# iwbn/flow-supervisor

Hardware: AMD Instinct MI355X
Metric: image-pairs/s fwd+bwd, 12 GRU iters, 436x1024 (higher is better)
Workload: dtype f32 (bf16x3 products); 1 GPU; RAFT full, 440x1024 (Sintel 436x1024 padded), 12 GRU iters, 4 pairs/GPU, train step = fwd + sequence loss + bwd + RCCL all-reduce + clip + AdamW; global_batch=4, parallelism=dp1, launch=hipGraph replay of the whole step

## Files before the change

flow_supervisor_amd/csrc/conv_pack.hip:

```cpp
#include "conv_common.hpp"

namespace {

struct PackArgs {
  float* w;
  float* wpk;
  int Cout, Cin, taps;
  int C[3]; int nsrc;
  int Ktot, rows;
  int mode, accumulate;
  int split;
};

__device__ __forceinline__ void store_packed(const PackArgs& a, int64_t e, float v) {
  if (!a.split) { a.wpk[e] = v; return; }
  const __bf16 h = (__bf16)v;
  const __bf16 l = (__bf16)(v - (float)h);
  __bf16* rec = reinterpret_cast<__bf16*>(a.wpk) + (e >> 5) * 64;
  rec[e & 31] = h;
  rec[32 + (e & 31)] = l;
}

__global__ __launch_bounds__(256) void pack_weight_kernel(PackArgs a) {
  const int64_t total = (int64_t)a.rows * a.Ktot;
  for (int64_t e = (int64_t)blockIdx.x * 256 + threadIdx.x; e < total; e += (int64_t)gridDim.x * 256) {
    const int n = (int)(e / a.Ktot);
    int k = (int)(e % a.Ktot);
    if (a.mode == 1) {
      const int cpad = ((a.Cout + 31) / 32) * 32;
      const int tp = k / cpad, c = k % cpad;
      float v = 0.f;
      if (c < a.Cout && n < a.Cin) v = a.w[((int64_t)c * a.Cin + n) * a.taps + (a.taps - 1 - tp)];
      store_packed(a, e, v);
    } else {
      int s = 0, coff = 0;
      for (; s < a.nsrc; ++s) {
        const int span = a.taps * (((a.C[s] + 31) / 32) * 32);
        if (k < span) break;
        k -= span; coff += a.C[s];
      }
      const int cpad = ((a.C[s] + 31) / 32) * 32;
      const int t = k / cpad, c = k % cpad;
      const bool ok = c < a.C[s] && n < a.Cout;
      if (a.mode == 0) {
        store_packed(a, e, ok ? a.w[((int64_t)n * a.Cin + coff + c) * a.taps + t] : 0.f);
      } else if (ok) {
        float* d = a.w + ((int64_t)n * a.Cin + coff + c) * a.taps + t;
        *d = a.accumulate ? *d + a.wpk[e] : a.wpk[e];
      }
    }
  }
}

using PackJob = fsraft_pack_job;
constexpr int PACK_JOBS = 16;
struct PackJobs { fsraft_pack_job j[PACK_JOBS]; };

__device__ __forceinline__ float* pack_elem(const PackJob& j, int n, int s, int c, int t) {
  int p = 0;
  while (p + 1 < j.npiece && n >= j.rows[p]) { n -= j.rows[p]; ++p; }
  float* w = j.w[p];
  if (j.flags & 2) {
    const int C = j.cin_full;
    const int sp = c / C, c0 = c % C;
    const int ky = 2 * (t >> 1) + (sp >> 1) - 1, kx = 2 * (t & 1) + (sp & 1) - 1;
    if (ky < 0 || kx < 0) return nullptr;
    return w + ((int64_t)n * C + c0) * 9 + ky * 3 + kx;
  }
  return w + ((int64_t)n * j.cin_full + j.srcOff[s] + c) * (j.kh * j.kw) + t;
}

__device__ __forceinline__ void pack_store(const PackJob& j, int Ktot, int rows, int n, int k, float v) {
  const int64_t e = (int64_t)n * Ktot + k;
  if (j.mode < 10) { j.wpk[e] = v; return; }
  const __bf16 h = (__bf16)v;
  const __bf16 l = (__bf16)(v - (float)h);
  __bf16* out = reinterpret_cast<__bf16*>(j.wpk);
  if (!(j.flags & 1)) {
    __bf16* rec = out + (e >> 5) * 64;
    rec[e & 31] = h;
    rec[32 + (e & 31)] = l;
    return;
  }
  const int nb = (rows + 31) / 32, kt = k >> 5, q = k & 31;
  const int64_t base = (((int64_t)kt * nb + (n >> 5)) * 2) ;
  const int sidx = (q >> 4) & 1, kh2 = (q >> 3) & 1, dw = (q >> 1) & 3, half = q & 1;
  const int64_t dh = ((((base + 0) * 2 + sidx) * 2 + kh2) * 32 + (n & 31)) * 4 + dw;
  const int64_t dl = ((((base + 1) * 2 + sidx) * 2 + kh2) * 32 + (n & 31)) * 4 + dw;
  out[dh * 2 + half] = h;
  out[dl * 2 + half] = l;
}

__global__ __launch_bounds__(256) void pack_jobs_kernel(PackJobs tab) {
  const PackJob& j = tab.j[blockIdx.y];
  const int taps = j.kh * j.kw;
  int cout = 0;
  for (int p = 0; p < j.npiece; ++p) cout += j.rows[p];
  if (j.mode == 3) {
    for (int e = blockIdx.x * 256 + threadIdx.x; e < cout; e += gridDim.x * 256) {
      int n = e, p = 0;
      while (p + 1 < j.npiece && n >= j.rows[p]) { n -= j.rows[p]; ++p; }
      j.wpk[e] = j.w[p][n];
    }
    return;
  }
  int cin = 0;
  for (int s = 0; s < j.nsrc; ++s) cin += j.srcC[s];
  const int m = j.mode % 10;
  int Ktot, rows;
  if (m == 1) { Ktot = taps * ((cout + 31) / 32 * 32); rows = cin; }
  else { Ktot = 0; for (int s = 0; s < j.nsrc; ++s) Ktot += taps * ((j.srcC[s] + 31) / 32 * 32); rows = cout; }
  const int rows_out = (j.flags & 1) ? (rows + 31) / 32 * 32 : rows;
  const int64_t total = (int64_t)rows_out * Ktot;
  for (int64_t e = (int64_t)blockIdx.x * 256 + threadIdx.x; e < total; e += (int64_t)gridDim.x * 256) {
    const int n = (int)(e / Ktot);
    int k = (int)(e % Ktot);
    if (m == 1) {
      const int cpad = (cout + 31) / 32 * 32;
      const int tp = k / cpad, c = k % cpad;
      float v = 0.f;
      if (c < cout && n < rows) {
        int s = 0, cs = n;
        while (s + 1 < j.nsrc && cs >= j.srcC[s]) { cs -= j.srcC[s]; ++s; }
        const float* q = pack_elem(j, c, s, cs, taps - 1 - tp);
        if (q) v = *q;
      }
      pack_store(j, Ktot, rows, n, k, v);
    } else {
      const int k0 = k;
      int s = 0;
      for (; s < j.nsrc; ++s) {
        const int span = taps * ((j.srcC[s] + 31) / 32 * 32);
        if (k < span) break;
        k -= span;
      }
      const int cpad = (j.srcC[s] + 31) / 32 * 32;
      const int t = k / cpad, c = k % cpad;
      const bool ok = c < j.srcC[s] && n < rows;
      float* q = ok ? pack_elem(j, n, s, c, t) : nullptr;
      if (m == 0) pack_store(j, Ktot, rows, n, k0, q ? *q : 0.f);
      else if (q) *q = j.accumulate ? *q + j.scale * j.wpk[e] : j.scale * j.wpk[e];
    }
  }
}

}

extern "C" int fsraft_pack_conv_weights(const fsraft_pack_job* jobs, int njobs, hipStream_t stream) {
  if (njobs < 0 || (njobs && !jobs)) return FS_ERR_ARG;
  for (int i = 0; i < njobs; ++i) {
    const fsraft_pack_job& j = jobs[i];
    const int m = j.mode;
    if (!(m == 0 || m == 1 || m == 2 || m == 3 || m == 10 || m == 11) || !j.wpk || j.npiece < 1 || j.npiece > 3) return FS_ERR_ARG;
    for (int p = 0; p < j.npiece; ++p) if (!j.w[p] || j.rows[p] < 1) return FS_ERR_ARG;
    if (m == 3) continue;
    if (j.nsrc < 1 || j.nsrc > 3 || j.kh < 1 || j.kw < 1 || j.cin_full < 1) return FS_ERR_ARG;
    if ((j.flags & 1) && m < 10) return FS_ERR_ARG;
    if ((j.flags & 2) && (j.kh != 2 || j.kw != 2 || j.nsrc != 1 || j.srcC[0] != 4 * j.cin_full || j.srcOff[0] != 0)) return FS_ERR_ARG;
    if (!(j.flags & 2)) for (int s = 0; s < j.nsrc; ++s) if (j.srcC[s] < 1 || j.srcOff[s] < 0 || j.srcOff[s] + j.srcC[s] > j.cin_full) return FS_ERR_ARG;
  }
  for (int i0 = 0; i0 < njobs; i0 += PACK_JOBS) {
    PackJobs tab{};
    const int n = njobs - i0 < PACK_JOBS ? njobs - i0 : PACK_JOBS;
    int64_t most = 0;
    for (int i = 0; i < n; ++i) {
      tab.j[i] = jobs[i0 + i];
      const fsraft_pack_job& j = tab.j[i];
      int64_t cout = 0, cin = 0;
      for (int p = 0; p < j.npiece; ++p) cout += j.rows[p];
      for (int s = 0; s < j.nsrc; ++s) cin += (j.srcC[s] + 31) / 32 * 32;
      const int64_t tot = j.mode == 3 ? cout : ((cout + 31) / 32 * 32) * ((cin + 31) / 32 * 32) * j.kh * j.kw;
      most = tot > most ? tot : most;
    }
    int blocks = (int)((most + 1023) / 1024);
    blocks = blocks < 1 ? 1 : (blocks > 512 ? 512 : blocks);
    hipLaunchKernelGGL(pack_jobs_kernel, dim3(blocks, n), dim3(256), 0, stream, tab);
  }
  return fs_launch_status();
}

extern "C" int fsraft_pack_conv_weight(float* w_oihw, float* wpk, int Cout, int Cin, int KH, int KW, const int* srcC,
                                       int nsrc, int mode, int accumulate, hipStream_t stream) {
  if (!w_oihw || !wpk || mode < 0 || (mode > 2 && mode != 10 && mode != 11)) return FS_ERR_ARG;
  PackArgs a{};
  a.split = mode >= 10;
  if (mode >= 10) mode -= 10;
  if (a.split && mode > 1) return FS_ERR_ARG;
  a.w = w_oihw; a.wpk = wpk; a.Cout = Cout; a.Cin = Cin; a.taps = KH * KW; a.mode = mode; a.accumulate = accumulate;
  if (mode == 1) {
    a.nsrc = 1; a.C[0] = Cout; a.C[1] = a.C[2] = 0;
    a.Ktot = a.taps * (((Cout + 31) / 32) * 32);
    a.rows = Cin;
  } else {
    if (!srcC || nsrc < 1 || nsrc > 3) return FS_ERR_ARG;
    int tot = 0;
    for (int s = 0; s < 3; ++s) { a.C[s] = s < nsrc ? srcC[s] : 0; tot += a.C[s]; }
    if (tot != Cin) return FS_ERR_ARG;
    a.nsrc = nsrc;
    a.Ktot = conv_ktot(srcC, nsrc, a.taps);
    a.rows = Cout;
  }
  const int64_t total = (int64_t)a.rows * a.Ktot;
  int blocks = (int)((total + 255) / 256 < 4096 ? (total + 255) / 256 : 4096);
  hipLaunchKernelGGL(pack_weight_kernel, dim3(blocks), dim3(256), 0, stream, a);
  return fs_launch_status();
}
```

Before: 111.1 image-pairs/s.

## Pack conv weights per 32-element record with vectorized stores and flat job grid

```diff
diff --git a/flow_supervisor_amd/csrc/conv_pack.hip b/flow_supervisor_amd/csrc/conv_pack.hip
--- a/flow_supervisor_amd/csrc/conv_pack.hip
+++ b/flow_supervisor_amd/csrc/conv_pack.hip
@@ -1,4 +1,5 @@
 #include "conv_common.hpp"
+#include <climits>
 
 namespace {
 
@@ -52,96 +53,149 @@
   }
 }
 
-using PackJob = fsraft_pack_job;
-constexpr int PACK_JOBS = 16;
-struct PackJobs { fsraft_pack_job j[PACK_JOBS]; };
-
-__device__ __forceinline__ float* pack_elem(const PackJob& j, int n, int s, int c, int t) {
-  int p = 0;
-  while (p + 1 < j.npiece && n >= j.rows[p]) { n -= j.rows[p]; ++p; }
-  float* w = j.w[p];
-  if (j.flags & 2) {
+constexpr int PACK_JOBS = 40;
+constexpr int PACK_RECS = 64;
+
+struct PackRec {
+  float* w[3];
+  float* wpk;
+  int rowEnd[3];
+  int cin_full, taps;
+  int srcC[3], srcOff[3];
+  int bits;
+  float scale;
+};
+struct PackTab {
+  PackRec j[PACK_JOBS];
+  int first[PACK_JOBS];
+  int njobs;
+};
+static_assert(sizeof(PackTab) <= 3840, "the job table has to fit the kernel argument segment");
+
+__device__ __forceinline__ int pick3(const int* a, int i) { return i == 0 ? a[0] : (i == 1 ? a[1] : a[2]); }
+__device__ __forceinline__ int ceil32(int v) { return (v + 31) / 32 * 32; }
+
+__device__ __forceinline__ float* pack_elem(const PackRec& j, int n, int s, int c, int t) {
+  const int p = (n >= j.rowEnd[0]) + (n >= j.rowEnd[1]);
+  float* w = p == 0 ? j.w[0] : (p == 1 ? j.w[1] : j.w[2]);
+  n -= p == 0 ? 0 : (p == 1 ? j.rowEnd[0] : j.rowEnd[1]);
+  if (j.bits & (2 << 7)) {
     const int C = j.cin_full;
     const int sp = c / C, c0 = c % C;
     const int ky = 2 * (t >> 1) + (sp >> 1) - 1, kx = 2 * (t & 1) + (sp & 1) - 1;
     if (ky < 0 || kx < 0) return nullptr;
     return w + ((int64_t)n * C + c0) * 9 + ky * 3 + kx;
   }
-  return w + ((int64_t)n * j.cin_full + j.srcOff[s] + c) * (j.kh * j.kw) + t;
-}
-
-__device__ __forceinline__ void pack_store(const PackJob& j, int Ktot, int rows, int n, int k, float v) {
-  const int64_t e = (int64_t)n * Ktot + k;
-  if (j.mode < 10) { j.wpk[e] = v; return; }
-  const __bf16 h = (__bf16)v;
-  const __bf16 l = (__bf16)(v - (float)h);
-  __bf16* out = reinterpret_cast<__bf16*>(j.wpk);
-  if (!(j.flags & 1)) {
-    __bf16* rec = out + (e >> 5) * 64;
-    rec[e & 31] = h;
-    rec[32 + (e & 31)] = l;
+  return w + ((int64_t)n * j.cin_full + pick3(j.srcOff, s) + c) * j.taps + t;
+}
+
+__device__ __forceinline__ uint32_t bf16_pair(__bf16 a, __bf16 b) {
+  return (uint32_t)__builtin_bit_cast(unsigned short, a) | ((uint32_t)__builtin_bit_cast(unsigned short, b) << 16);
+}
+
+__global__ __launch_bounds__(256) void pack_records_kernel(PackTab tab) {
+  const int blk = blockIdx.x;
+  int ji = 0, hi = tab.njobs - 1;
+  while (ji < hi) {
+    const int mid = (ji + hi + 1) >> 1;
+    if (tab.first[mid] <= blk) ji = mid; else hi = mid - 1;
+  }
+  const PackRec& j = tab.j[ji];
+  const int64_t r = (int64_t)(blk - tab.first[ji]) * PACK_RECS + (threadIdx.x >> 2);
+  const int l = threadIdx.x & 3;
+  const int nsrc = j.bits & 3, m = (j.bits >> 4) & 3, taps = j.taps, cout = j.rowEnd[2];
+  const bool split = j.bits & (1 << 6), frag = j.bits & (1 << 7), acc = j.bits & (1 << 9);
+  if (m == 3) {
+    for (int i = 0; i < 8; ++i) {
+      const int64_t e = r * 32 + l * 8 + i;
+      if (e >= cout) break;
+      const int n = (int)e, p = (n >= j.rowEnd[0]) + (n >= j.rowEnd[1]);
+      const float* w = p == 0 ? j.w[0] : (p == 1 ? j.w[1] : j.w[2]);
+      j.wpk[e] = w[n - (p == 0 ? 0 : (p == 1 ? j.rowEnd[0] : j.rowEnd[1]))];
+    }
     return;
   }
-  const int nb = (rows + 31) / 32, kt = k >> 5, q = k & 31;
-  const int64_t base = (((int64_t)kt * nb + (n >> 5)) * 2) ;
-  const int sidx = (q >> 4) & 1, kh2 = (q >> 3) & 1, dw = (q >> 1) & 3, half = q & 1;
-  const int64_t dh = ((((base + 0) * 2 + sidx) * 2 + kh2) * 32 + (n & 31)) * 4 + dw;
-  const int64_t dl = ((((base + 1) * 2 + sidx) * 2 + kh2) * 32 + (n & 31)) * 4 + dw;
-  out[dh * 2 + half] = h;
-  out[dl * 2 + half] = l;
-}
-
-__global__ __launch_bounds__(256) void pack_jobs_kernel(PackJobs tab) {
-  const PackJob& j = tab.j[blockIdx.y];
-  const int taps = j.kh * j.kw;
-  int cout = 0;
+  int cin = 0, kfwd = 0;
+  for (int s = 0; s < nsrc; ++s) { cin += pick3(j.srcC, s); kfwd += taps * ceil32(pick3(j.srcC, s)); }
+  const int cpo = ceil32(cout);
+  const int Ktot = m == 1 ? taps * cpo : kfwd, rows = m == 1 ? cin : cout;
+  const int rows_out = frag ? ceil32(rows) : rows;
+  const int KT = Ktot >> 5;
+  if (r >= (int64_t)rows_out * KT) return;
+  float* q[8];
+  int n, kt;
+  if (m == 1) {
+    const int per = rows_out * taps, ct = (int)(r / per), rem = (int)(r % per);
+    n = rem / taps;
+    const int tp = rem % taps;
+    kt = tp * (cpo >> 5) + ct;
+    int s = 0, cs = n;
+    while (s + 1 < nsrc && cs >= pick3(j.srcC, s)) { cs -= pick3(j.srcC, s); ++s; }
+    for (int i = 0; i < 8; ++i) {
+      const int c = ct * 32 + l * 8 + i;
+      q[i] = (c < cout && n < rows) ? pack_elem(j, c, s, cs, taps - 1 - tp) : nullptr;
+    }
+  } else {
+    n = (int)(r / KT);
+    kt = (int)(r % KT);
+    int k = kt * 32 + l * 8, s = 0;
+    for (; s + 1 < nsrc; ++s) {
+      const int span = taps * ceil32(pick3(j.srcC, s));
+      if (k < span) break;
+      k -= span;
+    }
+    const int cs = pick3(j.srcC, s), cpad = ceil32(cs);
+    const int t = k / cpad, c0 = k % cpad;
+    for (int i = 0; i < 8; ++i) q[i] = (c0 + i < cs && n < rows) ? pack_elem(j, n, s, c0 + i, t) : nullptr;
+  }
+  const int64_t e = (int64_t)n * Ktot + kt * 32 + l * 8;
+  if (m == 2) {
+    const float4 a = *reinterpret_cast<const float4*>(j.wpk + e), b = *reinterpret_cast<const float4*>(j.wpk + e + 4);
+    const float x[8] = {a.x, a.y, a.z, a.w, b.x, b.y, b.z, b.w};
+    for (int i = 0; i < 8; ++i)
+      if (q[i]) *q[i] = acc ? *q[i] + j.scale * x[i] : j.scale * x[i];
+    return;
+  }
+  float v[8];
+  for (int i = 0; i < 8; ++i) v[i] = q[i] ? *q[i] : 0.f;
+  if (!split) {
+    *reinterpret_cast<float4*>(j.wpk + e) = make_float4(v[0], v[1], v[2], v[3]);
+    *reinterpret_cast<float4*>(j.wpk + e + 4) = make_float4(v[4], v[5], v[6], v[7]);
+    return;
+  }
+  uint32_t h[4], lo[4];
+  for (int i = 0; i < 4; ++i) {
+    const __bf16 h0 = (__bf16)v[2 * i], h1 = (__bf16)v[2 * i + 1];
+    const __bf16 l0 = (__bf16)(v[2 * i] - (float)h0), l1 = (__bf16)(v[2 * i + 1] - (float)h1);
+    h[i] = bf16_pair(h0, h1);
+    lo[i] = bf16_pair(l0, l1);
+  }
+  uint32_t* out = reinterpret_cast<uint32_t*>(j.wpk);
+  int64_t dh, dl;
+  if (!frag) {
+    dh = (e >> 5) * 32 + l * 4;
+    dl = dh + 16;
+  } else {
+    const int nb = (rows + 31) / 32;
+    const int64_t base = ((int64_t)kt * nb + (n >> 5)) * 2;
+    dh = (((base + 0) * 4 + l) * 32 + (n & 31)) * 4;
+    dl = (((base + 1) * 4 + l) * 32 + (n & 31)) * 4;
+  }
+  *reinterpret_cast<uint4*>(out + dh) = make_uint4(h[0], h[1], h[2], h[3]);
+  *reinterpret_cast<uint4*>(out + dl) = make_uint4(lo[0], lo[1], lo[2], lo[3]);
+}
+
+int64_t pack_job_blocks(const fsraft_pack_job& j) {
+  int64_t cout = 0, cin = 0, kfwd = 0;
   for (int p = 0; p < j.npiece; ++p) cout += j.rows[p];
-  if (j.mode == 3) {
-    for (int e = blockIdx.x * 256 + threadIdx.x; e < cout; e += gridDim.x * 256) {
-      int n = e, p = 0;
-      while (p + 1 < j.npiece && n >= j.rows[p]) { n -= j.rows[p]; ++p; }
-      j.wpk[e] = j.w[p][n];
-    }
-    return;
-  }
-  int cin = 0;
-  for (int s = 0; s < j.nsrc; ++s) cin += j.srcC[s];
-  const int m = j.mode % 10;
-  int Ktot, rows;
-  if (m == 1) { Ktot = taps * ((cout + 31) / 32 * 32); rows = cin; }
-  else { Ktot = 0; for (int s = 0; s < j.nsrc; ++s) Ktot += taps * ((j.srcC[s] + 31) / 32 * 32); rows = cout; }
-  const int rows_out = (j.flags & 1) ? (rows + 31) / 32 * 32 : rows;
-  const int64_t total = (int64_t)rows_out * Ktot;
-  for (int64_t e = (int64_t)blockIdx.x * 256 + threadIdx.x; e < total; e += (int64_t)gridDim.x * 256) {
-    const int n = (int)(e / Ktot);
-    int k = (int)(e % Ktot);
-    if (m == 1) {
-      const int cpad = (cout + 31) / 32 * 32;
-      const int tp = k / cpad, c = k % cpad;
-      float v = 0.f;
-      if (c < cout && n < rows) {
-        int s = 0, cs = n;
-        while (s + 1 < j.nsrc && cs >= j.srcC[s]) { cs -= j.srcC[s]; ++s; }
-        const float* q = pack_elem(j, c, s, cs, taps - 1 - tp);
-        if (q) v = *q;
-      }
-      pack_store(j, Ktot, rows, n, k, v);
-    } else {
-      const int k0 = k;
-      int s = 0;
-      for (; s < j.nsrc; ++s) {
-        const int span = taps * ((j.srcC[s] + 31) / 32 * 32);
-        if (k < span) break;
-        k -= span;
-      }
-      const int cpad = (j.srcC[s] + 31) / 32 * 32;
-      const int t = k / cpad, c = k % cpad;
-      const bool ok = c < j.srcC[s] && n < rows;
-      float* q = ok ? pack_elem(j, n, s, c, t) : nullptr;
-      if (m == 0) pack_store(j, Ktot, rows, n, k0, q ? *q : 0.f);
-      else if (q) *q = j.accumulate ? *q + j.scale * j.wpk[e] : j.scale * j.wpk[e];
-    }
-  }
+  if (j.mode == 3) return ((cout + 31) / 32 + PACK_RECS - 1) / PACK_RECS;
+  const int64_t taps = (int64_t)j.kh * j.kw;
+  for (int s = 0; s < j.nsrc; ++s) { cin += j.srcC[s]; kfwd += taps * ((j.srcC[s] + 31) / 32); }
+  const bool dgrad = j.mode % 10 == 1;
+  int64_t rows = dgrad ? cin : cout;
+  if (j.flags & 1) rows = (rows + 31) / 32 * 32;
+  const int64_t recs = rows * (dgrad ? taps * ((cout + 31) / 32) : kfwd);
+  return (recs + PACK_RECS - 1) / PACK_RECS;
 }
 
 }
@@ -158,23 +212,32 @@
     if ((j.flags & 1) && m < 10) return FS_ERR_ARG;
     if ((j.flags & 2) && (j.kh != 2 || j.kw != 2 || j.nsrc != 1 || j.srcC[0] != 4 * j.cin_full || j.srcOff[0] != 0)) return FS_ERR_ARG;
     if (!(j.flags & 2)) for (int s = 0; s < j.nsrc; ++s) if (j.srcC[s] < 1 || j.srcOff[s] < 0 || j.srcOff[s] + j.srcC[s] > j.cin_full) return FS_ERR_ARG;
+    if ((reinterpret_cast<uintptr_t>(j.wpk) & 15) || (int64_t)j.kh * j.kw > (1 << 20) || pack_job_blocks(j) > INT_MAX / 2) return FS_ERR_ARG;
   }
   for (int i0 = 0; i0 < njobs; i0 += PACK_JOBS) {
-    PackJobs tab{};
-    const int n = njobs - i0 < PACK_JOBS ? njobs - i0 : PACK_JOBS;
-    int64_t most = 0;
-    for (int i = 0; i < n; ++i) {
-      tab.j[i] = jobs[i0 + i];
-      const fsraft_pack_job& j = tab.j[i];
-      int64_t cout = 0, cin = 0;
-      for (int p = 0; p < j.npiece; ++p) cout += j.rows[p];
-      for (int s = 0; s < j.nsrc; ++s) cin += (j.srcC[s] + 31) / 32 * 32;
-      const int64_t tot = j.mode == 3 ? cout : ((cout + 31) / 32 * 32) * ((cin + 31) / 32 * 32) * j.kh * j.kw;
-      most = tot > most ? tot : most;
-    }
-    int blocks = (int)((most + 1023) / 1024);
-    blocks = blocks < 1 ? 1 : (blocks > 512 ? 512 : blocks);
-    hipLaunchKernelGGL(pack_jobs_kernel, dim3(blocks, n), dim3(256), 0, stream, tab);
+    PackTab tab{};
+    tab.njobs = njobs - i0 < PACK_JOBS ? njobs - i0 : PACK_JOBS;
+    int64_t blocks = 0;
+    for (int i = 0; i < tab.njobs; ++i) {
+      const fsraft_pack_job& j = jobs[i0 + i];
+      PackRec& r = tab.j[i];
+      int sum = 0;
+      for (int p = 0; p < 3; ++p) {
+        r.w[p] = p < j.npiece ? j.w[p] : nullptr;
+        sum += p < j.npiece ? j.rows[p] : 0;
+        r.rowEnd[p] = sum;
+      }
+      r.wpk = j.wpk;
+      r.cin_full = j.cin_full; r.taps = j.kh * j.kw;
+      const int nsrc = j.mode == 3 ? 0 : j.nsrc;
+      for (int s = 0; s < 3; ++s) { r.srcC[s] = s < nsrc ? j.srcC[s] : 0; r.srcOff[s] = s < nsrc ? j.srcOff[s] : 0; }
+      r.bits = nsrc | (j.npiece << 2) | ((j.mode % 10) << 4) | ((j.mode >= 10 ? 1 : 0) << 6) | ((j.flags & 3) << 7) | ((j.accumulate ? 1 : 0) << 9);
+      r.scale = j.scale;
+      tab.first[i] = (int)blocks;
+      blocks += pack_job_blocks(j);
+      if (blocks > INT_MAX / 2) return FS_ERR_ARG;
+    }
+    if (blocks) hipLaunchKernelGGL(pack_records_kernel, dim3((unsigned)blocks), dim3(256), 0, stream, tab);
   }
   return fs_launch_status();
 }
```

Measured after the change: 111.5 image-pairs/s (median of 5 runs). Within noise of the previous version (+0.3%).
